# ekimb/mapquik

Hardware: AMD Instinct MI355X
Metric: Gbases/s mapped (sim CHM13v2-like HiFi, k=5 l=31 d=0.01) (higher is better)
Workload: dtype u64

## Files before the change

mapquik_amd/csrc/mq_capi_map.hpp:

```cpp
#pragma once

struct LaunchOpt {
    mq_kminmer *d_dump = nullptr;
    const uint64_t *d_dump_off = nullptr;
    uint32_t *d_dump_counts = nullptr;
    MatchRec *scratch_override = nullptr;
    uint32_t cap_override = 0;
    uint32_t grid_override = 0;
    uint32_t f16 = 0;
    const uint32_t *d_lens = nullptr;
    bool instrumented = false;
};

static int launch_map(mq_ctx *c, const uint8_t *d_bases, const uint64_t *d_offsets, uint32_t n, mq_hit *d_out, hipStream_t st,
                      const LaunchOpt &o = LaunchOpt()) {
    mq_index *idx = c->idx;
    if (n == 0) return MQ_OK;
    HIPCHK(hipMemsetAsync(c->d_counter, 0, 256, st));
    HIPCHK(hipEventRecord(c->ev0, st));
    SplitArgs A;
    A.bases = d_bases;
    A.offsets = d_offsets;
    A.lens = o.d_lens;
    A.n = n;
    A.P = idx->dp;
    A.mz_hash = c->mz_hash;
    A.mz_pos = c->mz_pos;
    A.mz_last = c->mz_last;
    A.mz_count = c->mz_count;
    A.mz_base = c->mz_base;
    A.pool_base = c->pool_base;
    A.pool_cap = c->pool_cap;
    A.f16 = o.f16 ? o.f16 : list_f16(idx);
    A.slack = LIST_SLACK;
    A.queue = c->queue;
    A.counters = c->d_counter;
    A.force_general = idx->force_general ? 1u : 0u;
    A.table = idx->table;
    A.mask = idx->nslots - 1;
    A.ref_lens = idx->d_ref_lens;
    A.scratch_all = o.scratch_override ? o.scratch_override : c->scratch;
    A.cap_matches = o.scratch_override ? o.cap_override : idx->cap_matches;
    A.out = d_out;
    A.dump = o.d_dump;
    A.dump_off = o.d_dump_off;
    A.dump_counts = o.d_dump_counts;
    A.stats64 = reinterpret_cast<unsigned long long *>(c->d_counter + 8);
    A.work = c->work;
    A.heavy_first = idx->heavy_first ? 1u : 0u;
    if (!idx->split) {
        if (n > WORK_ID_MASK) return set_err(MQ_EINVAL, "more than 2^30 - 1 reads in one batch");
        hipLaunchKernelGGL(order_reads_kernel, dim3((n + 255u) / 256u), dim3(256), 0, st, A);
        uint32_t grid = std::min<uint32_t>(idx->grid_fused, (n + MAP_WAVES - 1) / MAP_WAVES);
        if (o.grid_override) grid = std::min(grid, o.grid_override);
        const dim3 blk(64 * MAP_WAVES);
        if (idx->dp.variant) {
            if (o.instrumented) hipLaunchKernelGGL((map_kernel<64, true, true>), dim3(grid), blk, 0, st, A);
            else if (idx->chain_chunk == 4) hipLaunchKernelGGL((map_kernel<4, false, true>), dim3(grid), blk, 0, st, A);
            else hipLaunchKernelGGL((map_kernel<64, false, true>), dim3(grid), blk, 0, st, A);
        } else if (o.instrumented) hipLaunchKernelGGL((map_kernel<64, true>), dim3(grid), blk, 0, st, A);
        else if (idx->chain_chunk == 4) hipLaunchKernelGGL((map_kernel<4, false>), dim3(grid), blk, 0, st, A);
        else hipLaunchKernelGGL((map_kernel<64, false>), dim3(grid), blk, 0, st, A);
        HIPCHK(hipGetLastError());
        const uint32_t gd = grid;
        if (idx->dp.variant) {
            if (o.instrumented) hipLaunchKernelGGL((map_declined_kernel<64, true, true>), dim3(gd), blk, 0, st, A);
            else if (idx->chain_chunk == 4) hipLaunchKernelGGL((map_declined_kernel<4, false, true>), dim3(gd), blk, 0, st, A);
            else hipLaunchKernelGGL((map_declined_kernel<64, false, true>), dim3(gd), blk, 0, st, A);
        } else if (o.instrumented) hipLaunchKernelGGL((map_declined_kernel<64, true>), dim3(gd), blk, 0, st, A);
        else if (idx->chain_chunk == 4) hipLaunchKernelGGL((map_declined_kernel<4, false>), dim3(gd), blk, 0, st, A);
        else hipLaunchKernelGGL((map_declined_kernel<64, false>), dim3(gd), blk, 0, st, A);
        HIPCHK(hipGetLastError());
    } else {
        const uint32_t gs = std::min<uint32_t>(idx->grid_seed, (n + SEED_WAVES - 1) / SEED_WAVES);
        const char *ss = getenv("MQ_SEED_STOP");
        const int stop = ss ? atoi(ss) : 0;
        if (stop == 1) hipLaunchKernelGGL(seed_reads_kernel<1>, dim3(gs), dim3(64 * SEED_WAVES), 0, st, A);
        else if (stop == 2) hipLaunchKernelGGL(seed_reads_kernel<2>, dim3(gs), dim3(64 * SEED_WAVES), 0, st, A);
        else hipLaunchKernelGGL(seed_reads_kernel<0>, dim3(gs), dim3(64 * SEED_WAVES), 0, st, A);
        HIPCHK(hipGetLastError());
        const uint32_t gg = std::min<uint32_t>((uint32_t)idx->n_cu * 8u, n);
        hipLaunchKernelGGL(seed_general_kernel, dim3(gg), dim3(64), 0, st, A);
        HIPCHK(hipGetLastError());
        uint32_t gm = std::min<uint32_t>(idx->grid_map, (n + ML_WAVES - 1) / ML_WAVES);
        if (o.grid_override) gm = std::min(gm, o.grid_override);
        const dim3 blk(64 * ML_WAVES);
        if (o.instrumented) hipLaunchKernelGGL((map_lists_kernel<64, true>), dim3(gm), blk, 0, st, A);
        else if (idx->chain_chunk == 4) hipLaunchKernelGGL((map_lists_kernel<4, false>), dim3(gm), blk, 0, st, A);
        else hipLaunchKernelGGL((map_lists_kernel<64, false>), dim3(gm), blk, 0, st, A);
        HIPCHK(hipGetLastError());
    }
    HIPCHK(hipEventRecord(c->ev1, st));
    c->ev_valid = true;
    return MQ_OK;
}

static int redo_overflow(mq_ctx *c, const uint8_t *bases, const uint64_t *offsets, const uint32_t *lens, uint32_t n, mq_hit *out) {
    mq_index *idx = c->idx;
    std::vector<uint32_t> redo;
    for (uint32_t i = 0; i < n; ++i)
        if (out[i].status == MQ_HIT_OVERFLOW) redo.push_back(i);
    if (redo.empty()) return MQ_OK;
    uint64_t sub_max = 0;
    std::vector<uint64_t> so(redo.size() + 1, 0);
    for (size_t j = 0; j < redo.size(); ++j) {
        const uint64_t L = lens ? (uint64_t)lens[redo[j]] : offsets[redo[j] + 1] - offsets[redo[j]];
        so[j + 1] = so[j] + L;
        sub_max = std::max(sub_max, L);
    }
    const uint64_t sub_total = so.back();
    std::vector<uint8_t> sb(sub_total ? sub_total : 1);
    for (size_t j = 0; j < redo.size(); ++j) memcpy(sb.data() + so[j], bases + offsets[redo[j]], (size_t)(so[j + 1] - so[j]));
    const uint32_t cap = (uint32_t)std::max<uint64_t>(sub_max, 1);
    const uint32_t waves = std::max(MAP_WAVES, ML_WAVES);
    const uint32_t rgrid = (uint32_t)std::max<uint64_t>(1, std::min<uint64_t>(std::min(idx->grid_fused, idx->grid_map), (1ull << 30) / ((uint64_t)cap * sizeof(MatchRec) * waves)));
    int rc = ctx_ensure(c, (uint32_t)redo.size(), sub_total, 65536u);
    if (rc) return rc;
    MatchRec *big = nullptr;
// ... 537 lines not shown
```

mapquik_amd/csrc/mq_device.hpp:

```cpp
#pragma once
#include <hip/hip_runtime.h>
#include <stdint.h>

#include "../../include/mapquik_hip.h"
#include "../../include/mapquik_hip_diag.h"

namespace mq {

constexpr int WAVE = 64;
constexpr int RING = 512;
constexpr int MZ_CAP = 160;
constexpr int MAX_K = 32;
constexpr int MAX_L = 64;

struct DevParams {
    uint64_t bound;
    uint32_t k, l, use_hpc, c, s, g;
    uint32_t fold;
    uint32_t variant;
    uint32_t keep_none;
    uint32_t fast_kh;
};
template <bool VAR> __device__ __forceinline__ bool var_h32(const DevParams &P) { return VAR && (P.variant & MQ_SEEDVAR_HASH32) != 0; }
template <bool VAR> __device__ __forceinline__ bool var_pos_end(const DevParams &P) { return VAR && (P.variant & MQ_SEEDVAR_POS_RUN_END) != 0; }
template <bool VAR> __device__ __forceinline__ bool var_end_compressed(const DevParams &P) { return VAR && (P.variant & MQ_SEEDVAR_END_COMPRESSED) != 0; }
template <bool VAR> __device__ __forceinline__ bool var_rev_eq(const DevParams &P) { return VAR && (P.variant & MQ_SEEDVAR_REV_ON_EQUAL) != 0; }
template <bool VAR> __device__ __forceinline__ bool var_keep_none(const DevParams &P) { return VAR && P.keep_none != 0; }
template <bool VAR> __device__ __forceinline__ uint64_t list_hash(const DevParams &P, uint64_t h) { return var_h32<VAR>(P) ? (h & 0xFFFFFFFFull) : h; }

struct alignas(16) Entry {
    uint32_t start, end, offset, id_rc;
};
struct alignas(64) Bucket {
    unsigned long long key[2];
    Entry pay[2];
    uint32_t claims;
    uint32_t pad[3];
};
static_assert(sizeof(Bucket) == 64, "bucket size");
constexpr uint32_t ENTRY_DUP = 0x80000000u;
__device__ __forceinline__ bool entry_live(const Entry &e) { return e.end != 0u && !(e.id_rc & ENTRY_DUP); }
constexpr uint32_t SLOT_BYTES = 32;

struct alignas(8) RefKmm {
    unsigned long long hash;
    uint32_t start, end, offset, id_rc;
};
static_assert(sizeof(RefKmm) == 24, "RefKmm size");

struct alignas(16) MatchRec {
    uint32_t q_start, q_end, r_start, r_end, count, ref, rc, done;
};

struct WaveLds {
    unsigned long long mz_hash[MZ_CAP];
    uint32_t mz_pos[MZ_CAP];
    uint32_t mz_last[MZ_CAP];
    uint32_t ring_pos[RING];
    uint8_t ring_code[RING];
};

__device__ __forceinline__ void wave_sync() {
    __builtin_amdgcn_fence(__ATOMIC_RELEASE, "wavefront");
    __builtin_amdgcn_wave_barrier();
    __builtin_amdgcn_fence(__ATOMIC_ACQUIRE, "wavefront");
}
__device__ __forceinline__ uint32_t lane_id() {
    uint32_t x = __builtin_amdgcn_mbcnt_hi(~0u, __builtin_amdgcn_mbcnt_lo(~0u, 0u));
    asm volatile("" : "+v"(x));
    return x;
}
constexpr int MQ_N_CLK = 16;
#ifdef MQ_STAGE_CLOCKS
struct StageClkLds {
    unsigned long long acc[16][MQ_N_CLK];
    unsigned long long last[16];
};
__device__ __forceinline__ StageClkLds &mq_clk_lds() {
    __shared__ StageClkLds C;
    return C;
// ... 578 lines not shown
    if (n_cand == 0) return;
    if (n_cand > 1 && max_count == second_count) return;
    const bool rc = bfirst.rc != 0;
    const uint64_t q_start = bfirst.q_start;
    const uint64_t q_end = (uint64_t)blast.q_end - 1;
    uint64_t r_start, r_end;
    if (rc && b_len > 1) {
        r_start = blast.r_start;
        r_end = (uint64_t)bfirst.r_end - 1;
    } else {
        r_start = bfirst.r_start;
        r_end = (uint64_t)blast.r_end - 1;
    }
    const uint64_t r_len = ref_lens[b_ref];
    const uint64_t tail = q_len - q_end - 1;
    uint64_t frs, fre, exc_s, exc_e;
    if (!rc) {
        if (r_start >= q_start) { frs = r_start - q_start; exc_s = q_start; }
        else { frs = 0; exc_s = r_start; }
        if (r_end + tail <= r_len - 1) { fre = r_end + tail; exc_e = tail; }
        else { fre = r_len - 1; exc_e = r_len - r_end - 1; }
    } else {
        if (r_end + q_start <= r_len - 1) { fre = r_end + q_start; exc_s = q_start; }
        else { fre = r_len - 1; exc_s = r_len - r_end - 1; }
        if (r_start >= tail) { frs = r_start - tail; exc_e = tail; }
        else { frs = 0; exc_e = r_start; }
    }
    out.status = MQ_HIT_MAPPED;
    out.ref_id = b_ref;
    out.rc = rc ? 1u : 0u;
    out.mapq = b_mapq;
    const uint64_t qs64 = q_start - exc_s, qe64 = q_end + exc_e;
    out.q_start = (uint32_t)qs64;
    out.q_end = (uint32_t)qe64;
    out.q_start_hi = (uint32_t)(qs64 >> 32);
    out.q_end_hi = (uint32_t)(qe64 >> 32);
    out.r_start = (uint32_t)frs;
    out.r_end = (uint32_t)fre;
    out.score = b_score;
}

constexpr uint32_t MAP_LDS_RECS = 48;
static_assert(MAP_LDS_RECS <= 64, "records_to_scratch: one record per lane");
struct MapSink {
    const Bucket *__restrict__ table;
    uint64_t mask;
    const DevParams &P;
    MatchRec *__restrict__ scratch;
    uint32_t cap_matches;
    MatchRec *lds_rec;
    mq_kminmer *__restrict__ dump;
    uint32_t dump_cap;
    bool rev_eq;
    uint32_t kmm_count = 0;
    uint32_t n_matches = 0;
    bool c_open = false;
    MatchRec M = {};
    uint32_t c_hit = 0, c_id = 0, c_off = 0, c_sigma = 0;
    uint32_t probe_steps = 0;

    __device__ MapSink(const Bucket *t, uint64_t m, const DevParams &p, MatchRec *s, uint32_t cap, MatchRec *lr, mq_kminmer *d, uint32_t dc, bool re)
        : table(t), mask(m), P(p), scratch(s), cap_matches(cap), lds_rec(lr), dump(d), dump_cap(dc), rev_eq(re) {}
    __device__ __forceinline__ void put_rec(uint32_t i, const MatchRec &m) const {
        typedef uint32_t u32x4 __attribute__((ext_vector_type(4)));
        typedef __attribute__((address_space(3))) u32x4 lds_u4;
        if (i < MAP_LDS_RECS) {
            lds_u4 *d = (lds_u4 *)(&lds_rec[i]);
            d[0] = u32x4{m.q_start, m.q_end, m.r_start, m.r_end};
            d[1] = u32x4{m.count, m.ref, m.rc, m.done};
        } else if (i < cap_matches) {
            scratch[i] = m;
        }
    }
    __device__ __forceinline__ void records_to_scratch() const {
        const uint32_t n = n_matches < MAP_LDS_RECS ? n_matches : MAP_LDS_RECS, i = lane_id();
        if (i < n && i < cap_matches) scratch[i] = lds_rec[i];
    }

    __device__ __forceinline__ void batch_keys(const unsigned long long *mzh, const uint32_t *mzp, uint32_t base, bool act,
                                               uint64_t &key, bool &rev, uint32_t &q_start, uint32_t &q_end) const {
        const uint32_t i0 = base + lane_id();
        key = 0;
        rev = false;
        q_start = q_end = 0;
        if (act) {
            auto get = [&](uint32_t i) { return (uint64_t)mzh[i0 + i]; };
            const bool re = rev_eq, fk = P.fast_kh != 0;
            key = P.k == 5u ? kminmer_hash_fixed<5>(get, rev, re, fk) : P.k == 7u ? kminmer_hash_fixed<7>(get, rev, re, fk)
                  : P.k == 8u ? kminmer_hash_fixed<8>(get, rev, re, fk) : kminmer_hash(P.k, get, rev, re, fk);
            q_start = mzp[i0];
            q_end = mzp[i0 + P.k - 1] + P.l - 1u;
        }
    }

    __device__ __forceinline__ const Bucket *home_bucket(uint64_t key) const {
        return table + (key == 0 ? (mask + 1) >> 1 : (key & mask) >> 1);
    }
    template <int NB>
    __device__ __forceinline__ void probe_all(const uint64_t (&key)[NB], uint4 (&kk)[NB], uint32_t actbits, uint32_t &st) {
        st = 0;
        const uint64_t nb = (mask + 1) >> 1;
#pragma unroll
        for (int c = 0; c < NB; ++c) {
            if ((actbits >> c) & 1u) {
                const uint64_t k = key[c];
                const Bucket *B = home_bucket(k);
                uint32_t way, s2;
                if (k == 0) {
                    s2 = 1u;
                    way = 0;
                } else {
                    const uint32_t w0 = (uint32_t)k & (uint32_t)mask & 1u;
                    const uint64_t ka = u64_of(kk[c].x, kk[c].y), kb = u64_of(kk[c].z, kk[c].w);
                    const uint64_t kh = w0 ? kb : ka, kp = w0 ? ka : kb;
                    if (kh == k) { s2 = 1u; way = w0; }
                    else if (kh == 0) { s2 = 0u; way = 0; }
                    else if (kp == k) { s2 = 1u; way = w0 ^ 1u; probe_steps++; }
                    else if (kp == 0) { s2 = 0u; way = 0; probe_steps++; }
                    else { s2 = 3u; way = 0; probe_steps++; }
                }
                if (s2 == 1u) kk[c] = ld_u4(&B->pay[way]);
                st |= s2 << (2 * c);
            }
        }
#ifdef MQ_STAGE_MAP_SPLIT
        mq_clk(12);
#endif
        while (__ballot((st & 0xAAAAAAAAu) != 0)) {
            const bool walking = (st & 0xAAAAAAAAu) != 0;
            const uint32_t wc = walking ? ((uint32_t)__builtin_ctz(st & 0xAAAAAAAAu) >> 1) : 0xFFu;
            uint64_t k = 0;
#pragma unroll
            for (int c = 0; c < NB; ++c) k = wc == (uint32_t)c ? key[c] : k;
            uint64_t b = (k & mask) >> 1;
            uint4 res = make_uint4(0, 0, 0, 0);
            uint32_t s2 = walking ? 3u : 0u;
            while (__ballot(s2 == 3u)) {
                if (s2 == 3u) {
                    b = (b + 1) & (nb - 1);
                    const uint4 v = ld_u4(&table[b].key[0]);
// ... 214 lines not shown
```

mapquik_amd/csrc/mq_host_state.hpp:

```cpp
#pragma once


constexpr uint32_t MQ_MAX_REF_ID = 1u << 24;
static thread_local std::string g_err;
static int set_err(int code, const std::string &msg) {
    g_err = msg;
    return code;
}
#define HIPCHK(expr)                                                                                              \
    do {                                                                                                          \
        hipError_t _e = (expr);                                                                                   \
        if (_e != hipSuccess) {                                                                                   \
            char _b[512];                                                                                         \
            snprintf(_b, sizeof(_b), "%s failed: %s (%s:%d)", #expr, hipGetErrorString(_e), __FILE__, __LINE__);  \
            return set_err(_e == hipErrorOutOfMemory ? MQ_ENOMEM : MQ_EHIP, _b);                                  \
        }                                                                                                         \
    } while (0)

struct mq_index;

struct mq_ctx {
    mq_index *idx = nullptr;
    hipStream_t stream = nullptr;
    uint32_t *d_counter = nullptr;
// ... 26 lines not shown
    uint32_t *fx_tile_counts = nullptr, *fx_tile_off = nullptr;
    uint64_t fx_tile_counts_cap = 0, fx_tile_off_cap = 0;
    uint32_t *fx_nl = nullptr, *h_fx_nl = nullptr;
    uint64_t fx_nl_cap = 0, h_fx_nl_cap = 0;
    uint32_t *fx_info = nullptr, *h_fx_info = nullptr;
    uint8_t *h_fx_tail = nullptr;
    bool fx_pending = false;
    uint32_t fx_lpr = 2;
    const uint8_t *fx_buf = nullptr;
    uint32_t fx_begin = 0, fx_bytes = 0;
    bool pending = false;
    const uint8_t *p_bases = nullptr;
    const uint64_t *p_offsets = nullptr;
    const uint32_t *p_lens = nullptr;
    uint32_t p_n = 0;
    mq_hit *p_out = nullptr;
};

struct KmmChunk {
    RefKmm *d = nullptr;
    uint64_t n = 0, cap = 0;
};

struct mq_index {
    mq_params params;
    DevParams dp;
    int device = 0;
    int n_cu = 0;
    std::once_flag geometry_once;
    int geometry_rc = MQ_OK;
    std::mutex mu;
    std::map<uint32_t, std::pair<std::string, uint64_t>> refs;
    std::vector<KmmChunk> chunks;
    uint64_t n_kmm_total = 0;
    bool finalized = false;
    uint32_t table_factor = 0;
    Bucket *table = nullptr;
    uint64_t nslots = 0;
    uint64_t *d_ref_lens = nullptr;
    uint64_t n_unique = 0, n_keys = 0;
    uint8_t *bld_seq = nullptr;
    uint64_t bld_seq_cap = 0;
    unsigned long long *bld_seg_hash = nullptr, *bld_dense_hash = nullptr;
    uint32_t *bld_seg_pos = nullptr, *bld_dense_pos = nullptr;
    uint32_t *bld_seg_last = nullptr, *bld_dense_last = nullptr;
    uint64_t bld_seg_hash_cap = 0, bld_seg_pos_cap = 0, bld_dense_hash_cap = 0, bld_dense_pos_cap = 0, bld_seg_last_cap = 0, bld_dense_last_cap = 0;
    uint32_t *bld_counts = nullptr, *bld_queue = nullptr;
    uint64_t bld_counts_cap = 0, bld_queue_cap = 0;
    unsigned long long *bld_seg_off = nullptr;
    uint64_t bld_seg_off_cap = 0;
    unsigned long long *bld_info = nullptr;
    int grid_ref = 0;
    uint32_t grid_fused = 0, grid_seed = 0, grid_map = 0;
    uint32_t cap_matches = 0;
    bool split = false;
    bool force_general = false;
    bool heavy_first = true;
    int chain_chunk = 64;
    mq_ctx *def_ctx = nullptr;
    double t_add_ms = 0;
    std::mutex stg_mu;
    uint8_t *stg_buf = nullptr;
    uint64_t stg_bytes = 0;
    hipStream_t stg_stream = nullptr;
    std::vector<hipEvent_t> stg_events;
    uint64_t stg_issued = 0;
    std::thread rsv_thread;
    Bucket *rsv_table = nullptr;
    uint64_t rsv_nslots = 0;
    int rsv_err = 0;
    double table_alloc_ms = 0;
    double rsv_ms = 0;
};

static uint64_t table_slots_for(const mq_index *idx, uint64_t n_kmm) {
    const char *lf = getenv("MQ_TABLE_FACTOR");
    const uint64_t factor = lf && atoi(lf) >= 2 ? (uint64_t)atoi(lf) : idx->table_factor ? (uint64_t)idx->table_factor : 8ull;
    uint64_t nslots = 1024;
    while (nslots < factor * n_kmm) nslots <<= 1;
    return nslots;
}
static void rsv_join(mq_index *idx) {
    if (idx->rsv_thread.joinable()) idx->rsv_thread.join();
}

extern "C" {

const char *mq_last_error(void) { return g_err.c_str(); }
int mq_abi_version(void) { return MQ_ABI_VERSION; }

int mq_device_count(void) {
    int n = 0;
    hipError_t e = hipGetDeviceCount(&n);
    if (e != hipSuccess) {
        set_err(MQ_ENODEVICE, std::string("hipGetDeviceCount: ") + hipGetErrorString(e));
        return 0;
    }
    return n;
}

void mq_params_default(mq_params *p) {
    p->k = 5;
    p->l = 31;
    p->density = 0.01;
    p->use_hpc = 1;
    p->c = 4;
// ... 45 lines not shown
    return MQ_OK;
}

static size_t table_bytes_of(uint64_t nslots) { return (size_t)(nslots / 2 + 1) * sizeof(Bucket); }

static int alloc_table(mq_index *idx, uint64_t nslots) {
    if (idx->table) {
        HIPCHK(hipFree(idx->table));
        idx->table = nullptr;
    }
    if (nslots < 2) nslots = 2;
    const auto t0 = std::chrono::steady_clock::now();
    HIPCHK(hipMalloc((void **)&idx->table, table_bytes_of(nslots)));
    HIPCHK(hipMemset(idx->table, 0, table_bytes_of(nslots)));
    HIPCHK(hipDeviceSynchronize());
    idx->table_alloc_ms = std::chrono::duration<double, std::milli>(std::chrono::steady_clock::now() - t0).count();
    idx->nslots = nslots;
    return MQ_OK;
}

template <class T>
static int grow(T *&p, uint64_t &cap, uint64_t need) {
    if (need <= cap) return MQ_OK;
    if (p) HIPCHK(hipFree(p));
    p = nullptr;
    cap = 0;
    uint64_t nc = need + need / 4 + 64;
    HIPCHK(hipMalloc((void **)&p, nc * sizeof(T)));
    cap = nc;
    return MQ_OK;
}
template <class T>
static int grow_pinned(T *&p, uint64_t &cap, uint64_t need) {
    if (need <= cap) return MQ_OK;
    if (p) HIPCHK(hipHostFree(p));
    p = nullptr;
    cap = 0;
    uint64_t nc = need + need / 4 + 64;
    HIPCHK(hipHostMalloc((void **)&p, nc * sizeof(T), hipHostMallocDefault));
    cap = nc;
    return MQ_OK;
}

static int ensure_geometry_once(mq_index *idx) {
    auto occ_of = [&](const void *fn, int threads, int &occ) -> int {
        HIPCHK(hipOccupancyMaxActiveBlocksPerMultiprocessor(&occ, fn, threads, 0));
        if (occ < 1) occ = 1;
        if (occ > 8) occ = 8;
        const char *oe = getenv("MQ_OCC");
        if (oe && atoi(oe) >= 1 && atoi(oe) < occ) occ = atoi(oe);
        return MQ_OK;
    };
    int occ = 0, rc;
    {
        const void *fns[] = {(const void *)map_kernel<64, false, false>, (const void *)map_kernel<64, false, true>, (const void *)map_kernel<64, true, false>,
                             (const void *)map_kernel<64, true, true>, (const void *)map_kernel<4, false, false>, (const void *)map_kernel<4, false, true>,
                             (const void *)map_declined_kernel<64, false, false>, (const void *)map_declined_kernel<64, false, true>,
                             (const void *)map_declined_kernel<64, true, false>, (const void *)map_declined_kernel<64, true, true>,
                             (const void *)map_declined_kernel<4, false, false>, (const void *)map_declined_kernel<4, false, true>};
        int occ_min = 8;
        for (const void *fn : fns) {
            if ((rc = occ_of(fn, 64 * MAP_WAVES, occ))) return rc;
            occ_min = std::min(occ_min, occ);
        }
        occ = occ_min;
    }
    idx->grid_fused = (uint32_t)(occ * idx->n_cu);
    if ((rc = occ_of((const void *)seed_reads_kernel<0>, 64 * SEED_WAVES, occ))) return rc;
    idx->grid_seed = (uint32_t)(occ * idx->n_cu);
    if ((rc = occ_of((const void *)map_lists_kernel<64, false>, 64 * ML_WAVES, occ))) return rc;
    idx->grid_map = (uint32_t)(occ * idx->n_cu);
    const char *e = getenv("MQ_MATCH_CAP");
    idx->cap_matches = e ? (uint32_t)strtoul(e, nullptr, 10) : 2048u;
    if (idx->cap_matches < 1) idx->cap_matches = 1;
    return MQ_OK;
}

static int ensure_geometry(mq_index *idx) {
    std::call_once(idx->geometry_once, [idx] { idx->geometry_rc = ensure_geometry_once(idx); });
    return idx->geometry_rc;
}

static uint32_t list_f16(const mq_index *idx) {
    double d = idx->params.density;
    if (!(d > 0)) d = 0;
    double f = 4.0 * d + 1.0 / 512.0;
    if (f > 1.0) f = 1.0;
    const char *e = getenv("MQ_LIST_F16");
    if (e && atoi(e) >= 0) return (uint32_t)std::min(65536, atoi(e));
    return (uint32_t)std::ceil(f * 65536.0);
}
constexpr uint32_t LIST_SLACK = 64;

static int ctx_ensure(mq_ctx *c, uint32_t n, uint64_t total_bases, uint32_t f16) {
    mq_index *idx = c->idx;
    int rc = ensure_geometry(idx);
    if (rc) return rc;
    if (!c->d_counter) HIPCHK(hipMalloc((void **)&c->d_counter, 256));
    if (!c->ev0) {
        HIPCHK(hipEventCreate(&c->ev0));
        HIPCHK(hipEventCreate(&c->ev1));
    }
    {
        const size_t max_waves = std::max((size_t)idx->grid_fused * MAP_WAVES, (size_t)idx->grid_map * ML_WAVES);
        const size_t wpw = (size_t)std::max(MAP_WAVES, ML_WAVES);
        const size_t want = std::min(max_waves, ((size_t)n + wpw - 1) / wpw * wpw + wpw);
        if (want > c->scratch_waves) {
            if (c->scratch) HIPCHK(hipFree(c->scratch));
            c->scratch = nullptr;
            c->scratch_waves = 0;
            const size_t nw = std::min(max_waves, want + want / 4);
            HIPCHK(hipMalloc((void **)&c->scratch, nw * idx->cap_matches * sizeof(MatchRec)));
            c->scratch_waves = nw;
        }
    }
    if (n > c->reads_cap) {
        if (c->mz_count) HIPCHK(hipFree(c->mz_count));
        if (c->mz_base) HIPCHK(hipFree(c->mz_base));
        if (c->queue) HIPCHK(hipFree(c->queue));
        if (c->work) HIPCHK(hipFree(c->work));
// ... 118 lines not shown
```

mapquik_amd/csrc/mq_map_kernels.hpp:

```cpp
#pragma once


struct SplitArgs {
    const uint8_t *bases;
    const uint64_t *offsets;
    const uint32_t *lens;
    uint32_t n;
    DevParams P;
    unsigned long long *mz_hash;
    uint32_t *mz_pos;
    uint32_t *mz_last;
    uint32_t *mz_count;
    uint64_t *mz_base;
    uint64_t pool_base, pool_cap;
    uint32_t f16, slack;
    uint32_t *queue;
    uint32_t *counters;
    uint32_t force_general;
    const Bucket *table;
    uint64_t mask;
    const uint64_t *ref_lens;
    MatchRec *scratch_all;
    uint32_t cap_matches;
    mq_hit *out;
// ... 232 lines not shown
        }
        uint64_t seg_a = 0, seg_min_last = 0;
        uint64_t pos = 0, s = 0, d = 0;
        while (pos < len && next_clean_stretch(seq, len, pos, P.fold != 0, s, d)) {
            pos = d;
            if (d - s > 0xFFFFFF00ull) continue;
            if (s > seg_a) general(seg_a, s, seg_min_last);
            APre pre;
            SeedView V;
            V.first_prev = 4u;
            if (s > 0) {
                uint32_t b = seq[s - 1];
                if (P.fold && b - 'a' < 26u) b -= 32u;
                V.first_prev = b == 'A' ? 0u : b == 'C' ? 1u : b == 'T' ? 2u : b == 'G' ? 3u : 4u;
            }
            V.elig_end = (uint32_t)(((d - s) + 127u) & ~(uint64_t)63);
            V.pos_add = (uint32_t)s;
            V.more_after = 0u;
            const uint32_t left = cap_ > n_out ? cap_ - n_out : 0u;
            charge(0);
            const uint32_t c = seed_sequence_fast<0, true, VAR>(seq + s, (uint32_t)(d - s), P, T, SF, A.mz_hash + base_ + n_out, A.mz_pos + base_ + n_out, left, pre, false, V,
                                                                A.mz_last ? A.mz_last + base_ + n_out : nullptr);
            asm volatile("s_waitcnt vmcnt(0)" ::: "memory");
            wave_sync();
            charge(1);
            if (c == SD_NOT_FAST) {
                seg_a = s;
                seg_min_last = 0;
            } else {
                n_out += c;
                seg_a = heads_back(seq, s, d, P.l - 1u, P);
                seg_min_last = d;
            }
        }
        if (seg_a < len && seg_min_last < len) general(seg_a, len, seg_min_last);
        charge(0);
        return n_out;
    };
    uint32_t cnt = 0, cap_now = cap;
    for (int attempt = 0;; ++attempt) {
        cnt = pass(base, cap_now);
        if (cnt <= cap_now || attempt == 1) break;
        if (!pool_take(A, cnt, base)) {
            cnt = LIST_OVERFLOW;
            break;
        }
        cap_now = cnt;
        n_moved++;
    }
    return cnt;
}

#ifndef MQ_ML_NB
#define MQ_ML_NB 6
#endif
constexpr int ML_NB = MQ_ML_NB;
constexpr uint32_t ML_LIST_CAP = 64 * ML_NB + MAX_L;
static_assert(MAX_L >= 32, "k - 1 <= 31 entries of overlap between chunks");
struct MapListLds {
    unsigned long long h[ML_LIST_CAP];
    uint32_t p[ML_LIST_CAP];
    MatchRec rec[MAP_LDS_RECS];
};

__device__ __forceinline__ void store_hit(const SplitArgs &A, uint32_t r, const mq_hit &h) {
    if (lane_id() == 0) {
        A.out[r] = h;
        if (A.dump_counts) A.dump_counts[r] = h.n_kminmers;
    }
}

template <int CH, bool TIMING, bool VAR = true>
__device__ __forceinline__ void map_read(const SplitArgs &A, MapListLds &S, MatchRec *scratch, uint32_t r, uint64_t len, uint32_t cnt,
                                         uint64_t base, unsigned long long &t_steps, unsigned long long &t_lookups, mq_hit &h) {
    const uint32_t lane = lane_id();
    const DevParams &P = A.P;
    h.status = MQ_HIT_UNMAPPED;
    h.ref_id = h.rc = h.mapq = h.q_start = h.q_end = h.r_start = h.r_end = h.score = h.n_kminmers = h.q_start_hi = h.q_end_hi = 0;
    uint32_t n_kmm = 0;
    if (cnt == LIST_OVERFLOW) {
        h.status = MQ_HIT_OVERFLOW;
    } else if (cnt >= P.k) {
        mq_kminmer *d = nullptr;
        uint32_t dcap = 0;
        if (A.dump) {
            d = A.dump + A.dump_off[r];
            dcap = (uint32_t)(A.dump_off[r + 1] - A.dump_off[r]);
        }
        MapSink sink(A.table, A.mask, P, scratch, A.cap_matches, S.rec, d, dcap, var_rev_eq<VAR>(P));
        const unsigned long long *lh = A.mz_hash + base;
        const uint32_t *lp = A.mz_pos + base;
        const uint32_t chunk = 64u * (uint32_t)ML_NB + P.k - 1u;
        for (uint32_t g = 0; g + P.k <= cnt;) {
            const uint32_t have = cnt - g < chunk ? cnt - g : chunk;
            {
                unsigned long long hv[ML_NB + 1];
                uint32_t pv[ML_NB + 1];
#pragma unroll
                for (int j = 0; j <= ML_NB; ++j) {
                    const uint32_t i = lane + 64u * (uint32_t)j;
                    hv[j] = 0;
                    pv[j] = 0;
                    if (i < have) {
                        hv[j] = ld_sc1_u64(lh + g + i);
                        pv[j] = ld_sc1_u32(lp + g + i);
                    }
                }
#pragma unroll
                for (int j = 0; j <= ML_NB; ++j) {
                    const uint32_t i = lane + 64u * (uint32_t)j;
                    if (i < have) {
                        S.h[i] = hv[j];
                        S.p[i] = pv[j];
                    }
                }
            }
            wave_sync();
            mq_clk(5);
            uint32_t *mzq = (VAR && A.mz_last) ? reinterpret_cast<uint32_t *>(S.h) : nullptr;
            sink.template consume_list<ML_NB>(S.h, S.p, have, [&]() {
                if (mzq) {
                    const uint32_t *lq = A.mz_last + base + g;
                    wave_sync();
                    for (uint32_t i = lane; i < have; i += 64u) mzq[i] = ld_sc1_u32(lq + i);
                    wave_sync();
                }
            }, mzq);
            wave_sync();
            g += have - (P.k - 1u);
        }
        sink.finish_runs();
        n_kmm = sink.kmm_count;
        if (sink.n_matches > 0 && sink.n_matches <= MAP_LDS_RECS && sink.n_matches <= (uint32_t)CH) {
            wave_sync();
            MatchRec m0 = {};
            if (lane_id() < sink.n_matches) m0 = S.rec[lane_id()];
            mq_clk(8);
            chain_stage<CH>(S.rec, sink.n_matches, P, len, A.ref_lens, h, &m0);
        } else {
            if (sink.n_matches > 0 && sink.n_matches <= A.cap_matches) {
                wave_sync();
                sink.records_to_scratch();
            }
            if (sink.n_matches > A.cap_matches) {
                h.status = MQ_HIT_OVERFLOW;
            } else if (sink.n_matches > 0) {
                asm volatile("s_waitcnt vmcnt(0)" ::: "memory");
                wave_sync();
                mq_clk(8);
                chain_stage<CH>(scratch, sink.n_matches, P, len, A.ref_lens, h);
            }
        }
        if (TIMING) {
            t_steps += wave_sum_u32(sink.probe_steps);
            t_lookups += n_kmm;
        }
    }
    h.n_kminmers = n_kmm;
    mq_clk(9);
}

#ifndef MQ_MAP_WAVES
#define MQ_MAP_WAVES 8
#endif
#ifndef MQ_MAP_MIN_WAVES
#define MQ_MAP_MIN_WAVES 4
#endif
constexpr int MAP_WAVES = MQ_MAP_WAVES;

union MapWaveLds {
    SeedLds seed;
    WaveLds general;
    MapListLds map;
};

template <int CH, bool TIMING = false, bool VAR = false>
__global__ __launch_bounds__(64 * MAP_WAVES, MQ_MAP_MIN_WAVES) void map_kernel(const SplitArgs A) {
    __shared__ struct {
        SeedTables T;
        MapWaveLds SS[MAP_WAVES];
    } W;
    SeedTables &T = W.T;
    MapWaveLds(&SS)[MAP_WAVES] = W.SS;
    build_seed_tables(T, A.P.l, var_h32<VAR>(A.P));
    __syncthreads();
    const uint32_t lane = lane_id();
    const uint32_t wv = rdfirst(threadIdx.x >> 6);
    MapWaveLds &S = SS[wv];
    const size_t wave_gid = (size_t)blockIdx.x * MAP_WAVES + wv;
    MatchRec *scratch = A.scratch_all + wave_gid * A.cap_matches;
    const DevParams &P = A.P;
    const uint64_t o_base = A.offsets[0];
    uint32_t n_fast = 0, n_general = 0, n_moved = 0;
    unsigned long long t_steps = 0, t_lookups = 0;
#ifdef MQ_STAGE_CLOCKS
    if (lane == 0)
        for (int i = 0; i < MQ_N_CLK; ++i) mq_clk_lds().acc[wv][i] = 0;
    mq_clk(-1);
#endif
    const uint32_t nf = A.counters[WORK_NF] < WORK_FRONT_CAP ? A.counters[WORK_NF] : WORK_FRONT_CAP;
    const uint4 *work = A.work + (WORK_FRONT_CAP - nf);
    const uint32_t n_items = A.n + nf;
    uint32_t r = 0xFFFFFFFFu;
    uint64_t o0 = 0, len = 0;
    const uint32_t n_waves = gridDim.x * (uint32_t)MAP_WAVES;
    uint32_t own1 = (uint32_t)wave_gid, own2 = n_waves + (uint32_t)wave_gid;
    auto take_now = [&]() {
        for (;;) {
            uint32_t i;
            if (own1 != 0xFFFFFFFFu) {
                i = own1;
                own1 = 0xFFFFFFFFu;
            } else if (own2 != 0xFFFFFFFFu) {
                i = own2;
                own2 = 0xFFFFFFFFu;
            } else {
                i = 0;
                if (lane == 0) i = atomicAdd(&A.counters[0], 1u);
                i = rdfirst(i) + 2u * n_waves;
            }
            r = 0xFFFFFFFFu;
            if (i >= n_items) return;
            const uint4 d = work[i];
            if (d.w & WORK_SKIP) continue;
            r = d.w & WORK_ID_MASK;
            o0 = ((uint64_t)d.y << 32) | d.x;
            len = (uint64_t)d.z | ((uint64_t)((d.w >> 30) & 1u) << 32);
// ... 240 lines not shown
```

mapquik_amd/csrc/mq_seed.hpp:

```cpp
#pragma once
#include "mq_device.hpp"

namespace mq {

constexpr uint32_t SD_SR_RAW = 4096;
#ifndef MQ_SD_MAX_SR
#define MQ_SD_MAX_SR 3
#endif
constexpr uint32_t SD_MAX_SR = MQ_SD_MAX_SR;
constexpr uint32_t SD_TILE_RAW = SD_SR_RAW * SD_MAX_SR;
constexpr uint32_t SD_BLOCKS = SD_TILE_RAW / 64;
constexpr uint32_t SD_CODES_MAX = SD_TILE_RAW + MAX_L - 1;
constexpr uint32_t SD_LC_MAX = (SD_CODES_MAX + 63) / 64;
constexpr uint32_t SD_FLAG_WORDS = (SD_LC_MAX + 31) / 32;
constexpr uint32_t SD_CODES_DW = 4 * ((63 * SD_LC_MAX + 16 * ((SD_LC_MAX + 15) / 16) + MAX_L + 32) / 64 + 1);
static_assert((63 * SD_LC_MAX + 16 * ((SD_LC_MAX + 15) / 16) + MAX_L + 32) / 16 < SD_CODES_DW, "code stream read-ahead padding");
static_assert(2 * SD_CODES_MAX / 32 + 2 < SD_CODES_DW, "stage A writes three dwords from a piece pair's first");
#ifndef MQ_SD_OWNER_CAP
#define MQ_SD_OWNER_CAP 256
#endif
#ifndef MQ_SD_CROSS_PREFETCH
#define MQ_SD_CROSS_PREFETCH 1
#endif
constexpr bool SD_CROSS_PREFETCH = MQ_SD_CROSS_PREFETCH != 0;
constexpr uint32_t SD_OWNER_CAP = MQ_SD_OWNER_CAP;
static_assert(SD_BLOCKS <= 256, "block_of holds block numbers in a byte");

struct SeedTables {
    uint4 rot[32 * 16];
    uint4 rem[64];
    uint4 quad[256];
    uint16_t lut[1024];
};

constexpr uint32_t SD_BLOCK_OF_BYTES = (SD_CODES_MAX / 64 + 3 + 15) / 16 * 16;
struct SeedLds {
    uint32_t codes[SD_CODES_DW];
    uint8_t block_of[SD_BLOCK_OF_BYTES];
    unsigned long long heads[SD_BLOCKS];
    uint16_t cnt[SD_BLOCKS + 4];
    uint32_t flagw[SD_FLAG_WORDS * 64];
    uint32_t carry_codes[4];
    uint32_t carry_pos[64];
    uint16_t cand[SD_OWNER_CAP];
};

__device__ __forceinline__ uint64_t seed_of(uint32_t code, bool h32) {
    const uint64_t s = code == 0 ? 0x3c8bfbb395c60474ULL : code == 1 ? 0x3193c18562a02b4cULL : code == 2 ? 0x295549f54be24456ULL : 0x20323ed082572324ULL;
    return h32 ? dup_low(s) : s;
}

__device__ __forceinline__ void build_seed_tables(SeedTables &T, uint32_t l, bool h32) {
    auto seed_of = [h32](uint32_t code) { return mq::seed_of(code, h32); };
    for (uint32_t i = threadIdx.x; i < 1024; i += blockDim.x) {
        uint32_t prev = i & 3u, out = 0, n = 0, hb = 0;
        for (uint32_t m = 0; m < 4; ++m) {
            const uint32_t c = (i >> (2 + 2 * m)) & 3u;
            if (c != prev) {
                out |= c << (2 * n);
                n++;
                hb |= 1u << m;
            }
            prev = c;
        }
        T.lut[i] = (uint16_t)(out | ((2 * n) << 8) | (hb << 12));
    }
    for (uint32_t i = threadIdx.x; i < 32u * 16u; i += blockDim.x) {
        const uint32_t sft = i >> 4, o = i & 3u, in = (i >> 2) & 3u;
        const uint64_t f = rotr64(rotl64(seed_of(o), l) ^ seed_of(in), sft);
        const uint64_t r = rotl64(rotr64(seed_of(o ^ 2u), 1) ^ rotl64(seed_of(in ^ 2u), l - 1u), sft);
        T.rot[i] = h32 ? make_uint4((uint32_t)f, (uint32_t)r, (uint32_t)f, (uint32_t)r) : make_uint4((uint32_t)f, (uint32_t)(f >> 32), (uint32_t)r, (uint32_t)(r >> 32));
    }
    for (uint32_t i = threadIdx.x; i < 64; i += blockDim.x) {
        uint64_t f = 0, r = 0;
        for (uint32_t m = 0; m < (l & 3u); ++m) {
// ... 36 lines not shown
    __device__ __forceinline__ void roll(const uint4 tv) {
        const uint32_t nfhi = __builtin_amdgcn_alignbit(fhi, flo, 31), nflo = __builtin_amdgcn_alignbit(flo, fhi, 31);
        const uint32_t nrlo = __builtin_amdgcn_alignbit(rhi, rlo, 1), nrhi = __builtin_amdgcn_alignbit(rlo, rhi, 1);
        flo = nflo ^ tv.x;
        fhi = nfhi ^ tv.y;
        rlo = nrlo ^ tv.z;
        rhi = nrhi ^ tv.w;
    }
};

__device__ __forceinline__ uint4 load_piece(const uint8_t *__restrict__ seq, uint32_t len, uint32_t pos) {
    const uint32_t p = pos < len - 16u ? pos : len - 16u;
    return *reinterpret_cast<const uint4_unaligned *>(seq + p);
}
__device__ __forceinline__ uint4 fix_piece(const uint4 v, uint32_t len, uint32_t pos) {
    if (pos + 16u <= len) return v;
    const uint32_t fill = (v.w >> 24) * 0x01010101u;
    const uint32_t nv = pos < len ? len - pos : 0u;
    const uint32_t s = 16u - nv;
    uint32_t w0 = v.x, w1 = v.y, w2 = v.z, w3 = v.w;
    if (s & 4u) { w0 = w1; w1 = w2; w2 = w3; w3 = fill; }
    if (s & 8u) { w0 = w2; w1 = w3; w2 = fill; w3 = fill; }
    if (s & 16u) { w0 = fill; w1 = fill; w2 = fill; w3 = fill; }
    const uint32_t sb = s & 3u;
    return make_uint4(__builtin_amdgcn_alignbyte(w1, w0, sb), __builtin_amdgcn_alignbyte(w2, w1, sb),
                      __builtin_amdgcn_alignbyte(w3, w2, sb), __builtin_amdgcn_alignbyte(fill, w3, sb));
}

struct APre {
    uint4 nx0, nx1, nx2, nx3;
};
struct SeedView {
    uint32_t first_prev;
    uint32_t elig_end;
    uint32_t pos_add;
    uint32_t more_after;
};
__device__ __forceinline__ void stage_a_request(const uint8_t *__restrict__ seq, uint32_t len, uint32_t raw0, APre &pre) {
    const uint32_t pos = raw0 + lane_id() * 64u;
    pre.nx0 = load_piece(seq, len, pos);
    pre.nx1 = load_piece(seq, len, pos + 16u);
    pre.nx2 = load_piece(seq, len, pos + 32u);
    pre.nx3 = load_piece(seq, len, pos + 48u);
}

__device__ __forceinline__ bool seed_stage_a(const uint8_t *__restrict__ seq, uint32_t len, uint32_t raw0, uint32_t carry_n,
                                             uint32_t &carry_prev, bool use_hpc, bool fold, const SeedTables &T, SeedLds &S, uint32_t &n_codes,
                                             uint32_t &n_blocks, uint32_t &raw_end, APre &pre, bool first_is_head = true) {
    const uint32_t lane = lane_id();
    uint32_t n_sr = (len - raw0 + SD_SR_RAW - 1u) / SD_SR_RAW;
    if (n_sr > SD_MAX_SR) n_sr = SD_MAX_SR;
    const uint32_t tile_end = raw0 + n_sr * SD_SR_RAW;
    uint4 &nx0 = pre.nx0, &nx1 = pre.nx1, &nx2 = pre.nx2, &nx3 = pre.nx3;
    if (!SD_CROSS_PREFETCH && raw0 != 0) stage_a_request(seq, len, raw0, pre);
    static_assert(offsetof(SeedLds, block_of) == sizeof(uint32_t) * SD_CODES_DW && SD_CODES_DW % 4 == 0, "block_of is zeroed with the code stream");
    for (uint32_t i = lane * 4u; i < SD_CODES_DW + SD_BLOCK_OF_BYTES / 4u; i += 256u)
        *reinterpret_cast<uint4 *>(reinterpret_cast<uint32_t *>(&S) + i) = make_uint4(0, 0, 0, 0);
    wave_sync();
    if (lane < 4u && carry_n) S.codes[lane] = S.carry_codes[lane];
    uint32_t b2 = 2u * carry_n;
    uint32_t bad = 0;
    constexpr uint32_t S1 = 0x00430041u, S0 = 0x00470054u;
    for (uint32_t sr = 0; sr < n_sr; ++sr) {
        const uint32_t pos = raw0 + sr * SD_SR_RAW + lane * 64u;
        const bool more_sr = sr + 1u < n_sr || (SD_CROSS_PREFETCH && tile_end < len);
        if (raw0 + (sr + 1u) * SD_SR_RAW > len) {
            nx0 = fix_piece(nx0, len, pos);
            nx1 = fix_piece(nx1, len, pos + 16u);
            nx2 = fix_piece(nx2, len, pos + 32u);
            nx3 = fix_piece(nx3, len, pos + 48u);
        }
#ifdef MQ_STAGE_A_SPLIT
        if (sr == 0) mq_clk(raw0 == 0 ? 10 : 13);
        asm volatile("s_waitcnt vmcnt(0) lgkmcnt(0)" ::: "memory");
        mq_clk(sr == 0 ? (raw0 == 0 ? 0 : 14) : 12);
#endif
        uint32_t p[4];
        (void)more_sr;
        auto decode = [&](uint4 &nx, uint32_t j) {
            const uint32_t t0 = nx.x & 0x06060606u, t1 = nx.y & 0x06060606u, t2 = nx.z & 0x06060606u, t3 = nx.w & 0x06060606u;
            bad |= (__builtin_amdgcn_perm(S0, S1, t0) ^ nx.x) | (__builtin_amdgcn_perm(S0, S1, t1) ^ nx.y) |
                   (__builtin_amdgcn_perm(S0, S1, t2) ^ nx.z) | (__builtin_amdgcn_perm(S0, S1, t3) ^ nx.w);
            p[j] = pack16(t0, t1, t2, t3);
            nx = load_piece(seq, len, pos + SD_SR_RAW + 16u * j);
        };
        decode(nx0, 0);
        decode(nx1, 1);
        decode(nx2, 2);
        decode(nx3, 3);
        uint32_t out[4], n2[4], hb[4];
        if (use_hpc) {
            uint32_t pc = (uint32_t)__builtin_amdgcn_update_dpp(0, (int)(p[3] >> 30), 0x138, 0xf, 0xf, false);
            if (lane == 0) pc = (sr == 0 && raw0 == 0 && first_is_head) ? ((p[0] & 3u) ^ 1u) : carry_prev;
#pragma unroll
            for (int j = 0; j < 4; ++j) {
                const uint32_t q = (p[j] << 2) | pc;
                pc = p[j] >> 30;
                const uint32_t e0 = T.lut[q & 0x3FFu], e1 = T.lut[(q >> 8) & 0x3FFu], e2 = T.lut[(q >> 16) & 0x3FFu], e3 = T.lut[p[j] >> 22];
                uint32_t o = e0 & 0xFFu, sh = (e0 >> 8) & 15u;
                o |= (e1 & 0xFFu) << sh;
                sh += (e1 >> 8) & 15u;
                o |= (e2 & 0xFFu) << sh;
                sh += (e2 >> 8) & 15u;
                o |= (e3 & 0xFFu) << sh;
                out[j] = o;
                n2[j] = sh + ((e3 >> 8) & 15u);
                hb[j] = (e0 >> 12) | ((e1 >> 12) << 4) | ((e2 >> 12) << 8) | ((e3 >> 12) << 12);
// ... 502 lines not shown
                    const uint32_t t = s0 + 32u * w + (uint32_t)__ffs((int)g) - 1u;
                    if (has && at < SD_OWNER_CAP) S.cand[at] = (uint16_t)t;
                    at += has ? 1u : 0u;
                    g &= g - 1u;
                }
            }
        }
        wave_sync();
#ifdef MQ_STAGE_R_SPLIT
        mq_clk(13);
#endif
        const uint32_t r1 = total - r0 < SD_OWNER_CAP ? total : r0 + SD_OWNER_CAP;
        for (uint32_t i0 = r0; i0 < r1; i0 += 64u) {
            const uint32_t i = i0 + lane;
            if (i < r1) {
                const uint32_t j = S.cand[i - r0];
                const Hash2 wh = window_hash(T, S, P.l, j);
#ifdef MQ_STAGE_R_SPLIT
                asm volatile("s_waitcnt lgkmcnt(0)" ::: "memory");
                asm volatile("" ::"v"(wh.flo), "v"(wh.fhi), "v"(wh.rlo), "v"(wh.rhi));
                mq_clk(14);
#endif
                const uint32_t pos = seed_rawpos_batch(S, raw_base, carry_n, j);
                const uint64_t F = ((uint64_t)wh.fhi << 32) | wh.flo, R = ((uint64_t)wh.rhi << 32) | wh.rlo;
                const uint64_t hv = F < R ? F : R;
                if (hv > P.bound) inexact = true;
                const uint32_t dest = out_base + i;
                const bool listed = !VIEW || pos < V.elig_end;
                uint32_t rep = pos, lp = 0;
                if (var_pos_end<VAR>(P)) rep = seed_rawpos_batch(S, raw_base, carry_n, j + 1u) - 1u;
                if (var_end_compressed<VAR>(P)) lp = seed_rawpos_batch(S, raw_base, carry_n, j + P.l - 1u) + (VIEW ? V.pos_add : 0u);
                if (listed) out.put(dest, list_hash<VAR>(P, hv), VIEW ? rep + V.pos_add : rep, lp);
                if (VIEW) n_listed += (uint32_t)__popcll(__ballot(listed));
            }
#ifdef MQ_STAGE_R_SPLIT
            mq_clk(15);
#endif
        }
        wave_sync();
    }
    inexact = __ballot(inexact) != 0;
    return VIEW ? rdfirst(n_listed) : total;
}

constexpr uint32_t SD_NOT_FAST = 0xFFFFFFFFu;
__device__ __forceinline__ bool seed_fast_eligible(uint64_t len) { return len >= 16u && (len >> 32) == 0; }
template <int STOP = 0, bool VIEW = false, class Out = GlobalList, bool VAR = true>
__device__ __forceinline__ uint32_t seed_sequence_fast_to(const uint8_t *__restrict__ seq, uint32_t len, const DevParams &P, const SeedTables &T,
                                                          SeedLds &S, const Out &out, APre &pre, bool pre_valid, const SeedView &V = SeedView()) {
    const uint32_t lane = lane_id();
    uint32_t raw0 = 0, carry_n = 0, carry_prev = VIEW ? (V.first_prev & 3u) : 0u, n_out = 0;
    uint32_t halo_heads = 0, seg_heads = 0;
    if (!seed_fast_eligible(len)) return SD_NOT_FAST;
    if (!pre_valid) stage_a_request(seq, len, 0, pre);
    while (raw0 < len) {
        uint32_t n_codes = 0, n_blocks = 0, raw_end = 0;
        const bool ok = seed_stage_a(seq, len, raw0, carry_n, carry_prev, P.use_hpc != 0, P.fold != 0, T, S, n_codes, n_blocks, raw_end, pre,
                                     !VIEW || V.first_prev >= 4u);
        mq_clk(0);
        if (!ok) return SD_NOT_FAST;
        if (VIEW && V.more_after) {
            uint32_t c = 0, c0 = 0;
            for (uint32_t k = lane; k < n_blocks; k += 64u) {
                const uint32_t n = (uint32_t)__popcll(S.heads[k]);
                if (raw0 + 64u * k >= V.elig_end) c += n;
                else c0 += n;
            }
            halo_heads += wave_sum_u32(c);
            seg_heads += wave_sum_u32(c0);
        }
        const bool more = raw_end < len;
        if (STOP != 1 && n_codes >= P.l) {
            const uint32_t w_eff = n_codes - P.l + 1u;
            if (var_h32<VAR>(P)) seed_stage_b32(T, S, P, w_eff);
            else seed_stage_b(T, S, P, w_eff);
            mq_clk(1);
            if (STOP != 2) {
                bool inexact = false;
                n_out += seed_stage_r<VIEW, Out, VAR>(T, S, P, w_eff, n_blocks, n_codes, raw0, carry_n, out, n_out, inexact, V);
                mq_clk(2);
                if (inexact) return SD_NOT_FAST;
            }
        }
        if (more) {
            const uint32_t new_cn = n_codes < P.l - 1u ? n_codes : P.l - 1u;
            uint32_t cpos = 0, ccode = 0;
            if (lane < new_cn) cpos = seed_rawpos_batch(S, raw0, carry_n, n_codes - new_cn + lane);
            if (lane < 4u) {
                const uint32_t sb = 2u * (n_codes - new_cn) + 32u * lane;
                ccode = __builtin_amdgcn_alignbit(S.codes[(sb >> 5) + 1u], S.codes[sb >> 5], sb & 31u);
                const uint32_t keep = 2u * new_cn > 32u * lane ? 2u * new_cn - 32u * lane : 0u;
                ccode = keep >= 32u ? ccode : (ccode & ((1u << keep) - 1u));
            }
            wave_sync();
            if (lane < new_cn) S.carry_pos[lane] = cpos;
            if (lane < 4u) S.carry_codes[lane] = ccode;
            carry_n = new_cn;
        }
        wave_sync();
        raw0 = raw_end;
        mq_clk(3);
    }
    if (VIEW && V.more_after && halo_heads + 1u < P.l && seg_heads != 0u) return SD_NOT_FAST;
    return n_out;
}
template <int STOP = 0, bool VIEW = false, bool VAR = true>
__device__ __forceinline__ uint32_t seed_sequence_fast(const uint8_t *__restrict__ seq, uint32_t len, const DevParams &P, const SeedTables &T,
                                                       SeedLds &S, unsigned long long *__restrict__ mz_hash,
// ... 8 lines not shown
```

Baseline: 1372.

## Size map grid from the launched kernel pair and parametrize LDS on wave count

The fused map grid is now sized from the occupancy of the kernel pair actually launched (plus a separate grid for instrumented runs), not the minimum over all twelve template instantiations. The variant kernel is also selected when only fast_kh is set, and fast_kh is now carried through the MapSink. Several seeding and map-list constants (ML_NB, SD_MAX_SR, owner cap, cross prefetch) now scale down when MQ_MAP_WAVES exceeds 8, with static_asserts on the LDS budget. With the default of 8 waves, the main effect is a possibly larger grid if the slowest-occupancy instantiation is not the one launched, and the fast_kh routing through the variant path.

```diff
diff --git a/mapquik_amd/csrc/mq_capi_map.hpp b/mapquik_amd/csrc/mq_capi_map.hpp
--- a/mapquik_amd/csrc/mq_capi_map.hpp
+++ b/mapquik_amd/csrc/mq_capi_map.hpp
@@ -51,10 +51,11 @@
     if (!idx->split) {
         if (n > WORK_ID_MASK) return set_err(MQ_EINVAL, "more than 2^30 - 1 reads in one batch");
         hipLaunchKernelGGL(order_reads_kernel, dim3((n + 255u) / 256u), dim3(256), 0, st, A);
-        uint32_t grid = std::min<uint32_t>(idx->grid_fused, (n + MAP_WAVES - 1) / MAP_WAVES);
+        uint32_t grid = std::min<uint32_t>(o.instrumented ? idx->grid_instr : idx->grid_fused, (n + MAP_WAVES - 1) / MAP_WAVES);
         if (o.grid_override) grid = std::min(grid, o.grid_override);
         const dim3 blk(64 * MAP_WAVES);
-        if (idx->dp.variant) {
+        const bool var = idx->dp.variant != 0 || idx->dp.fast_kh != 0;
+        if (var) {
             if (o.instrumented) hipLaunchKernelGGL((map_kernel<64, true, true>), dim3(grid), blk, 0, st, A);
             else if (idx->chain_chunk == 4) hipLaunchKernelGGL((map_kernel<4, false, true>), dim3(grid), blk, 0, st, A);
             else hipLaunchKernelGGL((map_kernel<64, false, true>), dim3(grid), blk, 0, st, A);
@@ -63,7 +64,7 @@
         else hipLaunchKernelGGL((map_kernel<64, false>), dim3(grid), blk, 0, st, A);
         HIPCHK(hipGetLastError());
         const uint32_t gd = grid;
-        if (idx->dp.variant) {
+        if (var) {
             if (o.instrumented) hipLaunchKernelGGL((map_declined_kernel<64, true, true>), dim3(gd), blk, 0, st, A);
             else if (idx->chain_chunk == 4) hipLaunchKernelGGL((map_declined_kernel<4, false, true>), dim3(gd), blk, 0, st, A);
             else hipLaunchKernelGGL((map_declined_kernel<64, false, true>), dim3(gd), blk, 0, st, A);
diff --git a/mapquik_amd/csrc/mq_device.hpp b/mapquik_amd/csrc/mq_device.hpp
--- a/mapquik_amd/csrc/mq_device.hpp
+++ b/mapquik_amd/csrc/mq_device.hpp
@@ -26,6 +26,7 @@
 template <bool VAR> __device__ __forceinline__ bool var_end_compressed(const DevParams &P) { return VAR && (P.variant & MQ_SEEDVAR_END_COMPRESSED) != 0; }
 template <bool VAR> __device__ __forceinline__ bool var_rev_eq(const DevParams &P) { return VAR && (P.variant & MQ_SEEDVAR_REV_ON_EQUAL) != 0; }
 template <bool VAR> __device__ __forceinline__ bool var_keep_none(const DevParams &P) { return VAR && P.keep_none != 0; }
+template <bool VAR> __device__ __forceinline__ bool var_fast_kh(const DevParams &P) { return VAR && P.fast_kh != 0; }
 template <bool VAR> __device__ __forceinline__ uint64_t list_hash(const DevParams &P, uint64_t h) { return var_h32<VAR>(P) ? (h & 0xFFFFFFFFull) : h; }
 
 struct alignas(16) Entry {
@@ -710,6 +711,7 @@
     mq_kminmer *__restrict__ dump;
     uint32_t dump_cap;
     bool rev_eq;
+    bool fast_kh;
     uint32_t kmm_count = 0;
     uint32_t n_matches = 0;
     bool c_open = false;
@@ -717,8 +719,8 @@
     uint32_t c_hit = 0, c_id = 0, c_off = 0, c_sigma = 0;
     uint32_t probe_steps = 0;
 
-    __device__ MapSink(const Bucket *t, uint64_t m, const DevParams &p, MatchRec *s, uint32_t cap, MatchRec *lr, mq_kminmer *d, uint32_t dc, bool re)
-        : table(t), mask(m), P(p), scratch(s), cap_matches(cap), lds_rec(lr), dump(d), dump_cap(dc), rev_eq(re) {}
+    __device__ MapSink(const Bucket *t, uint64_t m, const DevParams &p, MatchRec *s, uint32_t cap, MatchRec *lr, mq_kminmer *d, uint32_t dc, bool re, bool fk)
+        : table(t), mask(m), P(p), scratch(s), cap_matches(cap), lds_rec(lr), dump(d), dump_cap(dc), rev_eq(re), fast_kh(fk) {}
     __device__ __forceinline__ void put_rec(uint32_t i, const MatchRec &m) const {
         typedef uint32_t u32x4 __attribute__((ext_vector_type(4)));
         typedef __attribute__((address_space(3))) u32x4 lds_u4;
@@ -743,7 +745,7 @@
         q_start = q_end = 0;
         if (act) {
             auto get = [&](uint32_t i) { return (uint64_t)mzh[i0 + i]; };
-            const bool re = rev_eq, fk = P.fast_kh != 0;
+            const bool re = rev_eq, fk = fast_kh;
             key = P.k == 5u ? kminmer_hash_fixed<5>(get, rev, re, fk) : P.k == 7u ? kminmer_hash_fixed<7>(get, rev, re, fk)
                   : P.k == 8u ? kminmer_hash_fixed<8>(get, rev, re, fk) : kminmer_hash(P.k, get, rev, re, fk);
             q_start = mzp[i0];
diff --git a/mapquik_amd/csrc/mq_host_state.hpp b/mapquik_amd/csrc/mq_host_state.hpp
--- a/mapquik_amd/csrc/mq_host_state.hpp
+++ b/mapquik_amd/csrc/mq_host_state.hpp
@@ -102,6 +102,7 @@
     unsigned long long *bld_info = nullptr;
     int grid_ref = 0;
     uint32_t grid_fused = 0, grid_seed = 0, grid_map = 0;
+    uint32_t grid_instr = 0;
     uint32_t cap_matches = 0;
     bool split = false;
     bool force_general = false;
@@ -253,20 +254,23 @@
         return MQ_OK;
     };
     int occ = 0, rc;
-    {
-        const void *fns[] = {(const void *)map_kernel<64, false, false>, (const void *)map_kernel<64, false, true>, (const void *)map_kernel<64, true, false>,
-                             (const void *)map_kernel<64, true, true>, (const void *)map_kernel<4, false, false>, (const void *)map_kernel<4, false, true>,
-                             (const void *)map_declined_kernel<64, false, false>, (const void *)map_declined_kernel<64, false, true>,
-                             (const void *)map_declined_kernel<64, true, false>, (const void *)map_declined_kernel<64, true, true>,
-                             (const void *)map_declined_kernel<4, false, false>, (const void *)map_declined_kernel<4, false, true>};
-        int occ_min = 8;
-        for (const void *fn : fns) {
-            if ((rc = occ_of(fn, 64 * MAP_WAVES, occ))) return rc;
-            occ_min = std::min(occ_min, occ);
-        }
-        occ = occ_min;
-    }
+    auto pair_occ = [&](const void *mk, const void *dk, int &o) -> int {
+        int a = 0, b = 0, r;
+        if ((r = occ_of(mk, 64 * MAP_WAVES, a)) || (r = occ_of(dk, 64 * MAP_WAVES, b))) return r;
+        o = std::min(a, b);
+        return MQ_OK;
+    };
+    const bool var = idx->dp.variant != 0 || idx->dp.fast_kh != 0;
+    if (var) rc = idx->chain_chunk == 4 ? pair_occ((const void *)map_kernel<4, false, true>, (const void *)map_declined_kernel<4, false, true>, occ)
+                                        : pair_occ((const void *)map_kernel<64, false, true>, (const void *)map_declined_kernel<64, false, true>, occ);
+    else rc = idx->chain_chunk == 4 ? pair_occ((const void *)map_kernel<4, false, false>, (const void *)map_declined_kernel<4, false, false>, occ)
+                                    : pair_occ((const void *)map_kernel<64, false, false>, (const void *)map_declined_kernel<64, false, false>, occ);
+    if (rc) return rc;
     idx->grid_fused = (uint32_t)(occ * idx->n_cu);
+    rc = var ? pair_occ((const void *)map_kernel<64, true, true>, (const void *)map_declined_kernel<64, true, true>, occ)
+             : pair_occ((const void *)map_kernel<64, true, false>, (const void *)map_declined_kernel<64, true, false>, occ);
+    if (rc) return rc;
+    idx->grid_instr = std::min(idx->grid_fused, (uint32_t)(occ * idx->n_cu));
     if ((rc = occ_of((const void *)seed_reads_kernel<0>, 64 * SEED_WAVES, occ))) return rc;
     idx->grid_seed = (uint32_t)(occ * idx->n_cu);
     if ((rc = occ_of((const void *)map_lists_kernel<64, false>, 64 * ML_WAVES, occ))) return rc;
diff --git a/mapquik_amd/csrc/mq_map_kernels.hpp b/mapquik_amd/csrc/mq_map_kernels.hpp
--- a/mapquik_amd/csrc/mq_map_kernels.hpp
+++ b/mapquik_amd/csrc/mq_map_kernels.hpp
@@ -308,7 +308,7 @@
 }
 
 #ifndef MQ_ML_NB
-#define MQ_ML_NB 6
+#define MQ_ML_NB (MQ_MAP_WAVES > 8 ? 3 : 6)
 #endif
 constexpr int ML_NB = MQ_ML_NB;
 constexpr uint32_t ML_LIST_CAP = 64 * ML_NB + MAX_L;
@@ -343,7 +343,7 @@
             d = A.dump + A.dump_off[r];
             dcap = (uint32_t)(A.dump_off[r + 1] - A.dump_off[r]);
         }
-        MapSink sink(A.table, A.mask, P, scratch, A.cap_matches, S.rec, d, dcap, var_rev_eq<VAR>(P));
+        MapSink sink(A.table, A.mask, P, scratch, A.cap_matches, S.rec, d, dcap, var_rev_eq<VAR>(P), var_fast_kh<VAR>(P));
         const unsigned long long *lh = A.mz_hash + base;
         const uint32_t *lp = A.mz_pos + base;
         const uint32_t chunk = 64u * (uint32_t)ML_NB + P.k - 1u;
@@ -416,11 +416,8 @@
     mq_clk(9);
 }
 
-#ifndef MQ_MAP_WAVES
-#define MQ_MAP_WAVES 8
-#endif
 #ifndef MQ_MAP_MIN_WAVES
-#define MQ_MAP_MIN_WAVES 4
+#define MQ_MAP_MIN_WAVES (MQ_MAP_WAVES / 2)
 #endif
 constexpr int MAP_WAVES = MQ_MAP_WAVES;
 
@@ -429,6 +426,11 @@
     WaveLds general;
     MapListLds map;
 };
+constexpr size_t MAP_LDS_BUDGET = 80u * 1024u;
+static_assert(sizeof(SeedTables) + MAP_WAVES * sizeof(MapWaveLds) <= MAP_LDS_BUDGET, "map_kernel's LDS: two workgroups per CU");
+static_assert(sizeof(SeedLds) <= (MAP_LDS_BUDGET - sizeof(SeedTables)) / MAP_WAVES, "a wave's tile (code stream, heads, cnt, block_of, flag words, carry, candidates)");
+static_assert(sizeof(MapListLds) <= (MAP_LDS_BUDGET - sizeof(SeedTables)) / MAP_WAVES, "a wave's staged list + the Match records held in LDS");
+static_assert(sizeof(WaveLds) <= (MAP_LDS_BUDGET - sizeof(SeedTables)) / MAP_WAVES, "the general seeder's per-wave LDS");
 
 template <int CH, bool TIMING = false, bool VAR = false>
 __global__ __launch_bounds__(64 * MAP_WAVES, MQ_MAP_MIN_WAVES) void map_kernel(const SplitArgs A) {
diff --git a/mapquik_amd/csrc/mq_seed.hpp b/mapquik_amd/csrc/mq_seed.hpp
--- a/mapquik_amd/csrc/mq_seed.hpp
+++ b/mapquik_amd/csrc/mq_seed.hpp
@@ -4,8 +4,11 @@
 namespace mq {
 
 constexpr uint32_t SD_SR_RAW = 4096;
+#ifndef MQ_MAP_WAVES
+#define MQ_MAP_WAVES 8
+#endif
 #ifndef MQ_SD_MAX_SR
-#define MQ_SD_MAX_SR 3
+#define MQ_SD_MAX_SR (MQ_MAP_WAVES > 8 ? 2 : 3)
 #endif
 constexpr uint32_t SD_MAX_SR = MQ_SD_MAX_SR;
 constexpr uint32_t SD_TILE_RAW = SD_SR_RAW * SD_MAX_SR;
@@ -17,10 +20,10 @@
 static_assert((63 * SD_LC_MAX + 16 * ((SD_LC_MAX + 15) / 16) + MAX_L + 32) / 16 < SD_CODES_DW, "code stream read-ahead padding");
 static_assert(2 * SD_CODES_MAX / 32 + 2 < SD_CODES_DW, "stage A writes three dwords from a piece pair's first");
 #ifndef MQ_SD_OWNER_CAP
-#define MQ_SD_OWNER_CAP 256
+#define MQ_SD_OWNER_CAP (MQ_MAP_WAVES > 8 ? 128 : 256)
 #endif
 #ifndef MQ_SD_CROSS_PREFETCH
-#define MQ_SD_CROSS_PREFETCH 1
+#define MQ_SD_CROSS_PREFETCH (MQ_MAP_WAVES > 8 ? 0 : 1)
 #endif
 constexpr bool SD_CROSS_PREFETCH = MQ_SD_CROSS_PREFETCH != 0;
 constexpr uint32_t SD_OWNER_CAP = MQ_SD_OWNER_CAP;
@@ -163,7 +166,6 @@
     if (n_sr > SD_MAX_SR) n_sr = SD_MAX_SR;
     const uint32_t tile_end = raw0 + n_sr * SD_SR_RAW;
     uint4 &nx0 = pre.nx0, &nx1 = pre.nx1, &nx2 = pre.nx2, &nx3 = pre.nx3;
-    if (!SD_CROSS_PREFETCH && raw0 != 0) stage_a_request(seq, len, raw0, pre);
     static_assert(offsetof(SeedLds, block_of) == sizeof(uint32_t) * SD_CODES_DW && SD_CODES_DW % 4 == 0, "block_of is zeroed with the code stream");
     for (uint32_t i = lane * 4u; i < SD_CODES_DW + SD_BLOCK_OF_BYTES / 4u; i += 256u)
         *reinterpret_cast<uint4 *>(reinterpret_cast<uint32_t *>(&S) + i) = make_uint4(0, 0, 0, 0);
@@ -772,8 +774,9 @@
     uint32_t raw0 = 0, carry_n = 0, carry_prev = VIEW ? (V.first_prev & 3u) : 0u, n_out = 0;
     uint32_t halo_heads = 0, seg_heads = 0;
     if (!seed_fast_eligible(len)) return SD_NOT_FAST;
-    if (!pre_valid) stage_a_request(seq, len, 0, pre);
+    if (SD_CROSS_PREFETCH && !pre_valid) stage_a_request(seq, len, 0, pre);
     while (raw0 < len) {
+        if (!SD_CROSS_PREFETCH) stage_a_request(seq, len, raw0, pre);
         uint32_t n_codes = 0, n_blocks = 0, raw_end = 0;
         const bool ok = seed_stage_a(seq, len, raw0, carry_n, carry_prev, P.use_hpc != 0, P.fold != 0, T, S, n_codes, n_blocks, raw_end, pre,
                                      !VIEW || V.first_prev >= 4u);
```

Result: no change. 1377 (median of 6 runs) (+0.4%).
